# zjtggssg/ST-GCN-AltFormer

Measured on AMD Instinct MI355X. Metric: clips/sec ST-GCN forward, higher is better.
Workload: dtype bf16x3 (fp32 operands split hi+lo bf16, 3 MFMAs, fp32 accumulate); 1 GPU; SHREC-graph stem forward: V=22, T=180, 256 clips/GPU (BASELINE configs[1] batch at 1 GPU; weak-scaled); clips_per_gpu=256, global_clips=256, T=180, V=22, workload_key=256x180x22 bf16x3 fused nctv, csrc_digest=4cb53548ea740e3b, math=bf16x3, fused=True, layout=nctv, parallelism=dp1, parity=1e-4 rel fp32 vs CPU oracle (tests/test_gpu_parity.py)

## Files before the change

### st-gcn-altformer_amd/csrc/kf6.h

```cpp
#pragma once

#include <type_traits>

#include "bf16_common.h"

namespace stgcn {

namespace {

using namespace bf16k;

constexpr int NP6 = 256;
constexpr int NT6 = 256;
constexpr int KT6 = 9;
constexpr int FRAG6 = 1024;
constexpr int PAIR6 = 16 * FRAG6;
constexpr int RING6 = 3 * PAIR6;
constexpr int EPI6 = 4096;

using f32x4 = __attribute__((ext_vector_type(4))) float;
typedef __attribute__((address_space(3))) void *lptr6_t;

__device__ __forceinline__ void dma16v6(const void *g, unsigned lds_addr) {
    const unsigned lds = __builtin_amdgcn_readfirstlane(lds_addr);
    asm volatile("s_mov_b32 m0, %1\n\ts_nop 0\n\tglobal_load_lds_dwordx4 %0, off" : : "v"(g), "s"(lds) : "memory", "m0");
}
template <int N>
__device__ __forceinline__ void vm_wait_keep() { asm volatile("s_waitcnt vmcnt(%0)" ::"n"(N) : "memory"); }

struct FragB6 { uint4 hi[4], lo[4]; };

template <int I, int N, class F>
__device__ __forceinline__ void static_for(F &&f) {
    if constexpr (I < N) {
        f(std::integral_constant<int, I>{});
        static_for<I + 1, N>(f);
    }
}

struct TileInfo6 {
    int n, Vh, j0, half;
    TileGeomB g;
};

__device__ __forceinline__ float relu1(float x) {
    float r;
    asm("v_max_f32_e32 %0, 0, %1" : "=v"(r) : "v"(x));
    return r;
}

#ifdef STGCN_ABLATION
#define V6_STAMP(var) unsigned long long var = 0; if (dbg) { asm volatile("s_memtime %0\n\ts_waitcnt lgkmcnt(0)" : "=s"(var) :: "memory"); }
#define V6_ACC(slot, a, b) if (dbg) { tsum[slot] += (b) - (a); }
#else
#define V6_STAMP(var)
#define V6_ACC(slot, a, b)
#endif


template <bool NT>
__device__ __forceinline__ void st_out4(float *p, const float4 &v) {
#ifndef V6_PLAIN_STORES
    if constexpr (NT) {
        using f32x4v = __attribute__((ext_vector_type(4))) float;
        __builtin_nontemporal_store(f32x4v{v.x, v.y, v.z, v.w}, reinterpret_cast<f32x4v *>(p));
        return;
    }
#endif
    *reinterpret_cast<float4 *>(p) = v;
}

template <int TERMS, bool BF16OUT, bool WIDE>
__global__ __launch_bounds__(NT6) void stem_bf16_v6_kernel(
    const uint4 *__restrict__ pfrag, const float *__restrict__ x, int xsc, int xsp, const float *__restrict__ W12,
    const uint4 *__restrict__ Wp, const float *__restrict__ shift, void *y, int C, int T, int V, int ROWS,
    int tiles_per_clip, int ntiles, int abl, unsigned long long *dbg, int V0, int tpc1) {
#ifdef STGCN_ABLATION
    unsigned long long tsum[8] = {0, 0, 0, 0, 0, 0, 0, 0};
#endif
    extern __shared__ __attribute__((aligned(16))) char smem6[];
    const int tid = threadIdx.x;
    const int lane = tid & 63;
    const int wave = __builtin_amdgcn_readfirstlane(tid >> 6);
    const int TV = T * V;
    const int nch = C / CCB;
    const int npairs = nch * KT6 / 2;
    const int img_bytes = ROWS * PXB;
    const int buf_bytes = img_bytes * (TERMS == 3 ? 2 : 1);
    uint4 *W12q = reinterpret_cast<uint4 *>(smem6);
    char *ring = smem6 + C * W12P * 4;
    char *buf0 = ring + RING6;
    char *buf1 = buf0 + buf_bytes;
    uint4 *Fs = reinterpret_cast<uint4 *>(buf0 + max(2 * buf_bytes, 4 * EPI6));
    const uint4 *Pf = (WIDE && TERMS == 3) ? reinterpret_cast<const uint4 *>(buf1) : Fs + 4 * ROWS;
    const unsigned lds0 = (unsigned)(size_t)(lptr6_t)smem6;
    const unsigned ring_lds = lds0 + (unsigned)(ring - smem6);
    const unsigned pf_lds = lds0 + (unsigned)(reinterpret_cast<const char *>(Pf) - smem6);

    const int cg = blockIdx.y;
    const uint4 *wsrc = Wp + ((size_t)(cg * 8 + 2 * wave) * npairs * 2) * 64 + lane;
    auto dma_frag = [&](int qsrc, int slot, int d) {
        const int bw = d >> 1, img = d & 1;
        dma16v6(wsrc + ((size_t)(bw * npairs + qsrc) * 2 + img) * 64, ring_lds + slot * PAIR6 + ((2 * wave + bw) * 2 + img) * FRAG6);
    };
    auto tile_info = [&](int tile) {
        TileInfo6 ti;
        ti.n = tile / tiles_per_clip;
        const int r = tile - ti.n * tiles_per_clip;
        int idx;
        if (r < 2 * tpc1) { ti.half = r & 1; idx = r >> 1; }
        else { ti.half = 0; idx = r - tpc1; }
        ti.Vh = ti.half ? V - V0 : V0;
        ti.j0 = ti.half ? V0 : 0;
        ti.g = tile_geom_b(idx, ti.Vh, KT6, 1, T, NP6);
        return ti;
    };
    auto dma_pfrag = [&](int tile) {
        if constexpr (WIDE) {
            const TileInfo6 ti = tile_info(tile);
            const uint4 *src = pfrag + ((size_t)ti.n * 48 + ti.half * 24) * 64 + lane;
#pragma unroll
            for (int i = 0; i < 6; ++i) dma16v6(src + (wave + 4 * i) * 64, pf_lds + (wave + 4 * i) * FRAG6);
        } else {
            const int n = tile / tiles_per_clip;
            const uint4 *src = pfrag + (size_t)n * 12 * 64 + lane;
#pragma unroll
            for (int i = 0; i < 3; ++i) dma16v6(src + (wave + 4 * i) * 64, pf_lds + (wave + 4 * i) * FRAG6);
        }
    };

    struct XRegs { float xa[WIDE ? 16 : 8]; float xp[3]; };
    auto load_x = [&](XRegs &xr, int tile, int u) {
        int ln = tid & 63;
        asm volatile("" : "+v"(ln));
        const int mb = u >> 1, hh = u & 1;
        TileInfo6 ti;
        if constexpr (WIDE) ti = tile_info(tile);
        else {
            ti.n = tile / tiles_per_clip;
            ti.g = tile_geom_b(tile - ti.n * tiles_per_clip, V, KT6, 1, T, NP6);
        }
        const int n = ti.n;
        const TileGeomB g = ti.g;
        const __amdgpu_buffer_rsrc_t rs = __builtin_amdgcn_make_buffer_rsrc(
            const_cast<float *>(x + (size_t)n * 3 * TV), 0, (unsigned)(3 * TV * 4), 0x00020000);
        const int tf = g.t_first - (KT6 - 1) / 2 + 4 * mb;
        if constexpr (WIDE) {
            const int k = ln & 3, t = tf + ((ln & 15) >> 2), v0 = 8 * (ln >> 4);
            const bool okr = (k < 3) & (t >= 0) & (t < T);
            unsigned base = (unsigned)((k * xsc + (t * V + v0) * xsp) * 4);
            asm volatile("" : "+v"(base));
#pragma unroll
            for (int j = 0; j < 16; ++j) {
                const int dv = (j & 7) + 32 * (j >> 3);
                const unsigned off = (okr & (v0 + dv < V)) ? base + (unsigned)(dv * xsp * 4) : 0x7ffffff0u;
                xr.xa[j] = __builtin_bit_cast(float, __builtin_amdgcn_raw_buffer_load_b32(rs, off, 0, 0));
            }
            const int t2 = tf + (ln >> 4), w = 16 * hh + (ln & 15);
            const bool ok = (t2 >= 0) & (t2 < T) & (w < ti.Vh);
            unsigned base2 = (unsigned)(((t2 * V + ti.j0 + w) * xsp) * 4);
            asm volatile("" : "+v"(base2));
#pragma unroll
            for (int k2 = 0; k2 < 3; ++k2) {
                const unsigned off = ok ? base2 + (unsigned)(k2 * xsc * 4) : 0x7ffffff0u;
                xr.xp[k2] = __builtin_bit_cast(float, __builtin_amdgcn_raw_buffer_load_b32(rs, off, 0, 0));
            }
        } else {
            {
                const int k = ln & 3, t = tf + ((ln & 15) >> 2), v0 = 8 * (ln >> 4);
                const bool okr = k < 3 && t >= 0 && t < T;
#pragma unroll
                for (int j = 0; j < 8; ++j) {
                    const unsigned off = (okr && v0 + j < V) ? (unsigned)((k * xsc + (t * V + v0 + j) * xsp) * 4) : 0x7ffffff0u;
                    xr.xa[j] = __builtin_bit_cast(float, __builtin_amdgcn_raw_buffer_load_b32(rs, off, 0, 0));
                }
            }
            {
// ... 57 lines not shown
        const bool valid = p < g.span && gi >= 0 && gi < T * Vh;
        const float one = valid ? 1.f : 0.f;
        const float fa[8] = {d[0][0] * one, d[0][1] * one, d[0][2] * one, d[1][0] * one,
                             d[1][1] * one, d[1][2] * one, d[2][0] * one, d[2][1] * one};
        const float fb[8] = {d[2][2] * one, xr.xp[0] * one, xr.xp[1] * one, xr.xp[2] * one, one, 0.f, 0.f, 0.f};
        uint4 ha, la, hb, lb;
        split8(fa, ha, la);
        split8(fb, hb, lb);
        if (w < Vh && p < ROWS) {
            Fs[p] = ha;
            Fs[(size_t)ROWS + p] = hb;
            Fs[(size_t)2 * ROWS + p] = la;
            Fs[(size_t)3 * ROWS + p] = lb;
        }
    };
    auto feature_phase = [&](int tile, const XRegs &x0, const XRegs &x1, const XRegs &x2) {
        TileInfo6 ti;
        if constexpr (WIDE) ti = tile_info(tile);
        else {
            ti.n = tile / tiles_per_clip;
            ti.Vh = V;
            ti.j0 = ti.half = 0;
            ti.g = tile_geom_b(tile - ti.n * tiles_per_clip, V, KT6, 1, T, NP6);
        }
        const TileGeomB &g = ti.g;
        const int need = min(ROWS, ((g.span + 15) >> 4) << 4);
        const int nun = (((need + ti.Vh - 1) / ti.Vh + 3) >> 2) * 2;
        const bool two = ti.Vh > 16;
        for (int u = wave; u < nun; u += 4) {
            if (!two && (u & 1)) continue;
            if (u == wave) feature_unit(ti, u, x0);
            else if (u == wave + 4) feature_unit(ti, u, x1);
            else if (u == wave + 8) feature_unit(ti, u, x2);
            else {
                XRegs xr;
                load_x(xr, tile, u);
                feature_unit(ti, u, xr);
            }
        }
    };

    const int pl = lane & 15, pg = lane >> 4;
    struct Prod { uint4 wh, wl, fb; f32x4 d; int p; };
    auto prod_load = [&](Prod &pr, int ch, int bi) {
        pr.p = bi * 16 + pl;
        pr.wh = W12q[(size_t)(pg & 1) * C + ch * CCB + pl];
        pr.wl = W12q[(size_t)(2 + (pg & 1)) * C + ch * CCB + pl];
        pr.fb = Fs[(size_t)pg * ROWS + pr.p];
    };
    auto prod_mfma = [&](Prod &pr) {
        const bf16x8 f = __builtin_bit_cast(bf16x8, pr.fb);
        pr.d = f32x4{0.f, 0.f, 0.f, 0.f};
        pr.d = __builtin_amdgcn_mfma_f32_16x16x32_bf16(__builtin_bit_cast(bf16x8, pr.wh), f, pr.d, 0, 0, 0);
        pr.d = __builtin_amdgcn_mfma_f32_16x16x32_bf16(__builtin_bit_cast(bf16x8, pr.wl), f, pr.d, 0, 0, 0);
    };
    auto prod_mfma_slots = [&](Prod &pr) {
        using u32x4 = __attribute__((ext_vector_type(4))) unsigned;
        const u32x4 wh = __builtin_bit_cast(u32x4, pr.wh), wl = __builtin_bit_cast(u32x4, pr.wl), fb = __builtin_bit_cast(u32x4, pr.fb);
        asm volatile("v_mfma_f32_16x16x32_bf16 %0, %1, %2, 0" : "=&v"(pr.d) : "v"(wh), "v"(fb));
        asm volatile("v_mfma_f32_16x16x32_bf16 %0, %1, %2, %0" : "+v"(pr.d) : "v"(wl), "v"(fb));
    };
    auto prod_finish = [&](char *buf, const Prod &pr) {
        const float v0 = relu1(pr.d[0]), v1 = relu1(pr.d[1]), v2 = relu1(pr.d[2]), v3 = relu1(pr.d[3]);
        const unsigned h0 = pack_bf16x2(v0, v1), h1 = pack_bf16x2(v2, v3);
        const int off = lds_off(pr.p, pg >> 1) + (pg & 1) * 8;
        *reinterpret_cast<uint2 *>(buf + off) = make_uint2(h0, h1);
        if constexpr (TERMS == 3) {
            const unsigned l0 = pack_bf16x2(v0 - bf16_lo_to_f32(h0), v1 - bf16_hi_to_f32(h0));
            const unsigned l1 = pack_bf16x2(v2 - bf16_lo_to_f32(h1), v3 - bf16_hi_to_f32(h1));
            *reinterpret_cast<uint2 *>(buf + img_bytes + off) = make_uint2(l0, l1);
        }
    };

    for (int e = tid; e < C * 2; e += NT6) {
        const int c = e >> 1, kh = e & 1;
        float w8[8];
#pragma unroll
        for (int i = 0; i < 8; ++i) w8[i] = W12[c * W12P + kh * 8 + i];
        uint4 hi, lo;
        split8(w8, hi, lo);
        W12q[(size_t)kh * C + c] = hi;
        W12q[(size_t)(2 + kh) * C + c] = lo;
    }
    int tile = blockIdx.x;
    {
        XRegs x0 = {}, x1 = {}, x2 = {};
        if (tile < ntiles) {
            dma_pfrag(tile);
            load_x(x0, tile, wave);
            load_x(x1, tile, wave + 4);
            load_x(x2, tile, wave + 8);
        }
#pragma unroll
        for (int d = 0; d < 4; ++d) { dma_frag(0, 0, d); dma_frag(1, 1, d); }
        vm_wait_keep<0>();
        __syncthreads();
        if (tile < ntiles) feature_phase(tile, x0, x1, x2);
        __syncthreads();
    }

    int slot0 = 0, slot2 = 2, q2 = 2 % npairs;
    const int sel = lane >> 5, chh = (lane >> 4) & 1;
    for (; tile < ntiles; tile += gridDim.x) {
        TileInfo6 ti;
        if constexpr (WIDE) ti = tile_info(tile);
        else {
            ti.n = tile / tiles_per_clip;
            ti.Vh = V;
            ti.j0 = ti.half = 0;
            ti.g = tile_geom_b(tile - ti.n * tiles_per_clip, V, KT6, 1, T, NP6);
        }
        const int n = ti.n;
        const TileGeomB g = ti.g;
        const int Vh = ti.Vh;
        const int nblk = (g.span + 15) >> 4;
        const int next_tile = tile + gridDim.x;

        V6_STAMP(t_0)
        for (int b = wave; b < nblk; b += 4) {
            Prod pr;
            prod_load(pr, 0, b);
            prod_mfma(pr);
            prod_finish(buf0, pr);
        }
        unsigned boff[KT6];
        {
            const int q = g.q0 + wave * 64 + (lane & 15);
            const int prow = q - g.t_first * Vh;
#pragma unroll
            for (int tap = 0; tap < KT6; ++tap) boff[tap] = (unsigned)lds_off(prow + tap * Vh, chh);
        }
        f32x4 acc[8][4];
#pragma unroll
        for (int mb = 0; mb < 8; ++mb)
#pragma unroll
            for (int nb = 0; nb < 4; ++nb) acc[mb][nb] = f32x4{0.f, 0.f, 0.f, 0.f};
        __syncthreads();
        V6_STAMP(t_1)
        V6_ACC(0, t_0, t_1)

        auto rd = [&](const char *p) { return *reinterpret_cast<const uint4 *>(p); };
        auto load_b = [&](FragB6 &b, auto l0_c, auto nb_c, auto lo_c) {
            constexpr int l0 = decltype(l0_c)::value, l1 = l0 + 1, nb = decltype(nb_c)::value;
            constexpr bool lo_img = decltype(lo_c)::value;
            const char *b0 = (l0 >= KT6 ? buf1 : buf0), *b1 = (l1 >= KT6 ? buf1 : buf0);
            const unsigned o0 = boff[l0 % KT6], o1 = boff[l1 % KT6];
            const char *p = (sel ? b1 : b0) + (sel ? o1 : o0) + (nb * 16 * PXB) + (lo_img ? img_bytes : 0);
            if constexpr (lo_img) b.lo[nb] = rd(p); else b.hi[nb] = rd(p);
        };
        using IC0 = std::integral_constant<int, 0>;
        FragB6 b_cur = {}, b_nxt = {};
        uint4 ah0n = rd(ring + slot0 * PAIR6 + lane * 16), al0n = rd(ring + slot0 * PAIR6 + lane * 16 + FRAG6);
        static_for<0, 4>([&](auto nb_c) {
            load_b(b_cur, IC0{}, nb_c, std::false_type{});
            if constexpr (TERMS == 3) load_b(b_cur, IC0{}, nb_c, std::true_type{});
        });
        const int nper = nch / 2;
        for (int per = 0; per < nper; ++per) {
            if constexpr (!WIDE)
                if (per + 1 == nper && next_tile < ntiles) dma_pfrag(next_tile);
            static_for<0, 9>([&](auto pi_c) {
                constexpr int pi = decltype(pi_c)::value;
                constexpr int l0 = 2 * pi;
                constexpr int win = pi <= 2 ? 0 : (pi >= 5 && pi <= 7 ? 1 : -1);
                constexpr int wpi = win == 0 ? pi : pi - 5;
                constexpr int npb = win < 0 ? 0 : (wpi < 2 ? 3 : 2);
// ... 12 lines not shown
                int poff = 0;
                constexpr int NM = 32 * TERMS;
                auto filler = [&](auto v_c) {
                    constexpr int v = decltype(v_c)::value;
                    if constexpr (v % 12 == 2 && v / 12 < 7) ah[(v / 12 + 1) & 1] = rd(aslot + ((v / 12 + 1) * 2) * FRAG6);
                    if constexpr (TERMS == 3 && v % 12 == 3 && v / 12 < 7) al[(v / 12 + 1) & 1] = rd(aslot + ((v / 12 + 1) * 2 + 1) * FRAG6);
                    if constexpr (v >= 40 && v < 48) {
                        constexpr int nb = (v - 40) / 2;
                        constexpr int ln = (l0 + 2) % 18;
                        using LN = std::integral_constant<int, ln>;
                        using NB = std::integral_constant<int, nb>;
                        if constexpr (v % 2 == 0) load_b(b_nxt, LN{}, NB{}, std::false_type{});
                        else if constexpr (TERMS == 3) load_b(b_nxt, LN{}, NB{}, std::true_type{});
                    }
                    if constexpr (npb > 0 && v >= 8 && (v - 8) / 28 < npb) {
                        constexpr int b = (v - 8) / 28, w = (v - 8) % 28;
                        auto piece = [&]() {
                            if constexpr (w == 0) {
                                pr.p = min(wave + 4 * (3 * wpi + b), nblk - 1) * 16 + pl;
                                pr.wh = W12q[(size_t)(pg & 1) * C + pch * CCB + pl];
                            }
                            if constexpr (w == 1) pr.wl = W12q[(size_t)(2 + (pg & 1)) * C + pch * CCB + pl];
                            if constexpr (w == 2) pr.fb = Fs[(size_t)pg * ROWS + pr.p];
                            if constexpr (w == 10) { if constexpr (TERMS == 3) prod_mfma_slots(pr); else prod_mfma(pr); }
                            if constexpr (w == 14) {
                                pv0 = relu1(pr.d[0]); pv1 = relu1(pr.d[1]); pv2 = relu1(pr.d[2]); pv3 = relu1(pr.d[3]);
                            }
                            if constexpr (w == 15) { ph0 = pack_bf16x2(pv0, pv1); ph1 = pack_bf16x2(pv2, pv3); }
                            if constexpr (w == 16) poff = lds_off(pr.p, pg >> 1) + (pg & 1) * 8;
                            if constexpr (w == 17) *reinterpret_cast<uint2 *>(pbuf + poff) = make_uint2(ph0, ph1);
                            if constexpr (TERMS == 3 && w == 18) { pv0 -= bf16_lo_to_f32(ph0); pv1 -= bf16_hi_to_f32(ph0); }
                            if constexpr (TERMS == 3 && w == 19) { pv2 -= bf16_lo_to_f32(ph1); pv3 -= bf16_hi_to_f32(ph1); }
                            if constexpr (TERMS == 3 && w == 20) { ph0 = pack_bf16x2(pv0, pv1); ph1 = pack_bf16x2(pv2, pv3); }
                            if constexpr (TERMS == 3 && w == 21) *reinterpret_cast<uint2 *>(pbuf + img_bytes + poff) = make_uint2(ph0, ph1);
                        };
                        constexpr bool has_work = w <= 2 || w == 10 || (w >= 14 && w <= 17) || (TERMS == 3 && w >= 18 && w <= 21);
                        if constexpr (has_work) piece();
                    }
                    if constexpr (v >= 4 && v < 8) dma_frag(q2, slot2, v - 4);
                    if constexpr (v == 88) ah0n = rd(anext);
                    if constexpr (TERMS == 3 && v == 89) al0n = rd(anext + FRAG6);
                };
                static_for<0, NM>([&](auto i_c) {
                    constexpr int i = decltype(i_c)::value;
                    constexpr int mb = i / (4 * TERMS), nb = (i / TERMS) % 4, term = i % TERMS;
                    const bf16x8 a_h = __builtin_bit_cast(bf16x8, ah[mb & 1]), b_h = __builtin_bit_cast(bf16x8, b_cur.hi[nb]);
                    if constexpr (TERMS == 3) {
                        const bf16x8 a_l = __builtin_bit_cast(bf16x8, al[mb & 1]), b_l = __builtin_bit_cast(bf16x8, b_cur.lo[nb]);
                        if constexpr (term == 0) acc[mb][nb] = __builtin_amdgcn_mfma_f32_16x16x32_bf16(a_h, b_l, acc[mb][nb], 0, 0, 0);
                        else if constexpr (term == 1) acc[mb][nb] = __builtin_amdgcn_mfma_f32_16x16x32_bf16(a_l, b_h, acc[mb][nb], 0, 0, 0);
                        else acc[mb][nb] = __builtin_amdgcn_mfma_f32_16x16x32_bf16(a_h, b_h, acc[mb][nb], 0, 0, 0);
                    } else {
                        acc[mb][nb] = __builtin_amdgcn_mfma_f32_16x16x32_bf16(a_h, b_h, acc[mb][nb], 0, 0, 0);
                    }
                    if constexpr (term == TERMS - 1) asm volatile("" : "+a"(acc[mb][nb]));
#ifndef V6_NOFILL
                    static_for<i * (96 / NM), (i + 1) * (96 / NM)>(filler);
#endif
                    __builtin_amdgcn_sched_barrier(0);
                });
                b_cur = b_nxt;
                V6_STAMP(t_s1)
                V6_ACC((pi == 4 ? 6 : (pi == 0 ? 7 : (pi == 3 ? 5 : 4))), t_p0, t_s1)
                vm_wait_keep<0>();
                __syncthreads();
                V6_STAMP(t_s2)
                V6_ACC(2, t_s1, t_s2)
                slot0 = slot1;
                slot2 = slot2 == 2 ? 0 : slot2 + 1;
                q2 = q2 + 1 == npairs ? 0 : q2 + 1;
            });
        }
        vm_wait_keep<0>();
        V6_STAMP(t_2)
        V6_ACC(1, t_1, t_2)

        if constexpr (WIDE)
            if (next_tile < ntiles) dma_pfrag(next_tile);
        XRegs xn0, xn1, xn2;
        load_x(xn0, min(next_tile, ntiles - 1), wave);
        load_x(xn1, min(next_tile, ntiles - 1), wave + 4);
        load_x(xn2, min(next_tile, ntiles - 1), wave + 8);
        __builtin_amdgcn_sched_barrier(0);
        float *stg = reinterpret_cast<float *>(buf0 + wave * EPI6);
        const int qw = g.q0 + wave * 64;
        const bool full = g.q0 + NP6 - 1 <= g.q_last;
        if constexpr (WIDE) {
            auto clip_pixel = [&](int q) { const int t = q / Vh; return t * V + ti.j0 + (q - t * Vh); };
            if (abl & OPT_OUT_NTVC) {
                unsigned pt[4];
                bool pok[4];
#pragma unroll
                for (int it = 0; it < 4; ++it) {
                    const int q = qw + it * 16 + (lane >> 2);
                    pok[it] = q <= g.q_last;
                    pt[it] = (unsigned)(clip_pixel(min(q, g.q_last)) * C + 4 * (lane & 3));
                }
#pragma unroll
                for (int mb = 0; mb < 8; ++mb) {
                    const int ob = cg * 128 + mb * 16;
                    const float4 sh4 = *reinterpret_cast<const float4 *>(shift + ob + 4 * (lane >> 4));
#pragma unroll
                    for (int nb = 0; nb < 4; ++nb) {
                        const int px = nb * 16 + (lane & 15);
                        const float4 v = make_float4(fmaxf(acc[mb][nb][0] + sh4.x, 0.f), fmaxf(acc[mb][nb][1] + sh4.y, 0.f),
                                                     fmaxf(acc[mb][nb][2] + sh4.z, 0.f), fmaxf(acc[mb][nb][3] + sh4.w, 0.f));
                        *reinterpret_cast<float4 *>(stg + px * 16 + (((lane >> 4) ^ (px & 3)) << 2)) = v;
                    }
                    const size_t tbase = (size_t)n * TV * C + ob;
#pragma unroll
                    for (int it = 0; it < 4; ++it) {
                        const int idx = it * 64 + lane, px = idx >> 2, sl = idx & 3;
                        const float4 v = *reinterpret_cast<const float4 *>(stg + px * 16 + ((sl ^ (px & 3)) << 2));
                        if (pok[it]) {
                            if constexpr (BF16OUT)
                                *reinterpret_cast<uint2 *>(reinterpret_cast<unsigned short *>(y) + tbase + pt[it]) =
                                    make_uint2(pack_bf16x2(v.x, v.y), pack_bf16x2(v.z, v.w));
                            else
                                st_out4<false>(reinterpret_cast<float *>(y) + tbase + pt[it], v);
                        }
                    }
                }
            } else {
                const int qp = qw + 2 * (lane & 31);
                const bool pok = qp <= g.q_last;
                const unsigned lterm = (unsigned)((lane >> 5) * TV + clip_pixel(min(qp, g.q_last)));
#pragma unroll
                for (int mb = 0; mb < 8; ++mb) {
                    const int ob = cg * 128 + mb * 16;
                    const float4 sh4 = *reinterpret_cast<const float4 *>(shift + ob + 4 * (lane >> 4));
                    const float shv[4] = {sh4.x, sh4.y, sh4.z, sh4.w};
#pragma unroll
                    for (int nb = 0; nb < 4; ++nb)
#pragma unroll
                        for (int r = 0; r < 4; ++r)
                            stg[(4 * (lane >> 4) + r) * 64 + nb * 16 + (lane & 15)] = fmaxf(acc[mb][nb][r] + shv[r], 0.f);
                    const size_t tbase = ((size_t)n * C + ob) * TV;
#pragma unroll
                    for (int it = 0; it < 8; ++it) {
                        const float2 v = *reinterpret_cast<const float2 *>(stg + (it * 2 + (lane >> 5)) * 64 + 2 * (lane & 31));
                        const size_t sbase = tbase + (size_t)(it * 2) * TV;
                        if (pok) {
                            if constexpr (BF16OUT)
                                *reinterpret_cast<unsigned *>(reinterpret_cast<unsigned short *>(y) + sbase + lterm) = pack_bf16x2(v.x, v.y);
                            else
                                *reinterpret_cast<float2 *>(reinterpret_cast<float *>(y) + sbase + lterm) = v;
                        }
                    }
                }
            }
        } else if (abl & OPT_OUT_NTVC) {
            const unsigned lterm = (unsigned)((lane >> 2) * C + 4 * (lane & 3));
#pragma unroll
            for (int mb = 0; mb < 8; ++mb) {
                const int ob = cg * 128 + mb * 16;
                const float4 sh4 = *reinterpret_cast<const float4 *>(shift + ob + 4 * (lane >> 4));
#pragma unroll
                for (int nb = 0; nb < 4; ++nb) {
                    const int px = nb * 16 + (lane & 15);
                    const float4 v = make_float4(fmaxf(acc[mb][nb][0] + sh4.x, 0.f), fmaxf(acc[mb][nb][1] + sh4.y, 0.f),
                                                 fmaxf(acc[mb][nb][2] + sh4.z, 0.f), fmaxf(acc[mb][nb][3] + sh4.w, 0.f));
                    *reinterpret_cast<float4 *>(stg + px * 16 + (((lane >> 4) ^ (px & 3)) << 2)) = v;
                }
                const size_t tbase = ((size_t)n * TV + qw) * C + ob;
#pragma unroll
                for (int it = 0; it < 4; ++it) {
                    const int idx = it * 64 + lane, px = idx >> 2, sl = idx & 3;
                    const float4 v = *reinterpret_cast<const float4 *>(stg + px * 16 + ((sl ^ (px & 3)) << 2));
                    if (full || qw + px <= g.q_last) {
                        if constexpr (BF16OUT) {
                            unsigned short *yb = reinterpret_cast<unsigned short *>(y) + tbase + (size_t)(it * 16) * C;
                            *reinterpret_cast<uint2 *>(yb + lterm) = make_uint2(pack_bf16x2(v.x, v.y), pack_bf16x2(v.z, v.w));
                        } else {
                            float *yb = reinterpret_cast<float *>(y) + tbase + (size_t)(it * 16) * C;
                            st_out4<true>(yb + lterm, v);
                        }
                    }
                }
            }
        } else {
            const unsigned lterm = (unsigned)((lane >> 4) * TV + 4 * (lane & 15));
            const int c4l = 4 * (lane & 15);
#pragma unroll
            for (int mb = 0; mb < 8; ++mb) {
                const int ob = cg * 128 + mb * 16;
                const float4 sh4 = *reinterpret_cast<const float4 *>(shift + ob + 4 * (lane >> 4));
                const float shv[4] = {sh4.x, sh4.y, sh4.z, sh4.w};
#pragma unroll
                for (int nb = 0; nb < 4; ++nb)
#pragma unroll
                    for (int r = 0; r < 4; ++r)
                        stg[(4 * (lane >> 4) + r) * 64 + nb * 16 + (lane & 15)] = fmaxf(acc[mb][nb][r] + shv[r], 0.f);
                const size_t tbase = ((size_t)n * C + ob) * TV + qw;
                const bool al16 = ((tbase & 3) == 0) && (TV % 4 == 0);
#pragma unroll
                for (int it = 0; it < 4; ++it) {
                    const float4 v = *reinterpret_cast<const float4 *>(stg + (it * 4 + (lane >> 4)) * 64 + c4l);
                    const size_t sbase = tbase + (size_t)(it * 4) * TV;
                    if (full && al16) {
                        if constexpr (BF16OUT)
                            *reinterpret_cast<uint2 *>(reinterpret_cast<unsigned short *>(y) + sbase + lterm) =
                                make_uint2(pack_bf16x2(v.x, v.y), pack_bf16x2(v.z, v.w));
                        else
                            st_out4<true>(reinterpret_cast<float *>(y) + sbase + lterm, v);
                    } else {
                        const float e4[4] = {v.x, v.y, v.z, v.w};
#pragma unroll
                        for (int e = 0; e < 4; ++e)
                            if (qw + c4l + e <= g.q_last) store_out<BF16OUT>(y, sbase + lterm + e, e4[e]);
                    }
                }
            }
        }
        V6_STAMP(t_3)
        V6_ACC(3, t_2, t_3)
        if (next_tile < ntiles) {
            if constexpr (WIDE) {
                vm_wait_keep<0>();
                __syncthreads();
            }
            feature_phase(next_tile, xn0, xn1, xn2);
            V6_STAMP(t_4)
            __syncthreads();
        }
        V6_STAMP(t_5)
    }
#ifdef STGCN_ABLATION
    if (dbg && lane == 0 && blockIdx.x < 8 && blockIdx.y == 0)
        for (int i = 0; i < 8; ++i) dbg[(blockIdx.x * 8 + wave) * 8 + i] = tsum[i];
#endif
}

struct V6Plan {
    int rows = 0, tiles_per_clip = 0;
    size_t lds = 0;
    int v0 = 0, tpc1 = 0;
};

inline int v6_rows(int T, int Vh, int K) {
    int dt = ceil_div(NP6 - 1, Vh);
    if (dt > T - 1) dt = T - 1;
    const int span = (dt + K) * Vh;
    if (ceil_div(ceil_div(span, 16), 4) > 8) return 0;
    return (span + 15) / 16 * 16;
}

inline bool plan_v6_narrow(int C, int T, int V, int K, int terms, V6Plan &pl) {
    if (K != KT6 || C % 128 != 0 || V > 32) return false;
    const int rows = v6_rows(T, V, K);
    if (rows == 0) return false;
    const size_t buf = (size_t)rows * PXB * (terms == 3 ? 2 : 1);
    const size_t img = 2 * buf > (size_t)4 * EPI6 ? 2 * buf : (size_t)4 * EPI6;
    pl.lds = (size_t)C * W12P * 4 + RING6 + img + (size_t)rows * 64 + 12 * FRAG6;
    if (pl.lds > (size_t)kLdsBytes) return false;
    pl.rows = rows;
    pl.tiles_per_clip = ceil_div(T * V, NP6);
    return true;
}

inline bool plan_v6_wide(int C, int T, int V, int K, int terms, V6Plan &pl) {
    const int v0 = stem_wide_split(V);
    if (K != KT6 || C % 128 != 0 || v0 == 0) return false;
    const int r0 = v6_rows(T, v0, K), r1 = v6_rows(T, V - v0, K);
    if (r0 == 0 || r1 == 0) return false;
    const int rows = r0 > r1 ? r0 : r1;
    const size_t buf = (size_t)rows * PXB * (terms == 3 ? 2 : 1);
    const size_t img = 2 * buf > (size_t)4 * EPI6 ? 2 * buf : (size_t)4 * EPI6;
    if (terms == 3 && buf < (size_t)24 * FRAG6) return false;
    pl.lds = (size_t)C * W12P * 4 + RING6 + img + (size_t)rows * 64 + (terms == 3 ? 0 : 24 * FRAG6);
    if (pl.lds > (size_t)kLdsBytes) return false;
    pl.rows = rows;
    pl.v0 = v0;
    pl.tpc1 = ceil_div(T * (V - v0), NP6);
    pl.tiles_per_clip = ceil_div(T * v0, NP6) + pl.tpc1;
    return pl.tiles_per_clip - pl.tpc1 >= pl.tpc1;
}

template <bool WIDE>
bool stem_v6_form_supported(int C, int T, int V, int K, unsigned flags) {
    const unsigned math = flags & STGCN_MATH_MASK;
    if (math != STGCN_MATH_BF16X3 && math != STGCN_MATH_BF16) return false;
    const int terms = math == STGCN_MATH_BF16X3 ? 3 : 1;
    V6Plan pl;
    return T >= 1 && (WIDE ? plan_v6_wide(C, T, V, K, terms, pl) : plan_v6_narrow(C, T, V, K, terms, pl));
}

template <int TERMS, bool WIDE>
int launch_v6(const uint4 *pf, const float *x, int xsc, int xsp, const float *W12, const uint4 *Wq, const float *shift, void *y,
              int N, int C, int T, int V, const V6Plan &pl, bool bf16out, int opt, int num_cu, hipStream_t st) {
    const int ntiles = N * pl.tiles_per_clip;
    const dim3 grid(ntiles < num_cu ? ntiles : num_cu, C / 128, 1);
    auto kern = bf16out ? stem_bf16_v6_kernel<TERMS, true, WIDE> : stem_bf16_v6_kernel<TERMS, false, WIDE>;
    STGCN_HIP_CHECK(allow_lds(kern, pl.lds));
    hipLaunchKernelGGL(kern, grid, dim3(NT6), pl.lds, st, pf, x, xsc, xsp, W12, Wq, shift, y, C, T, V, pl.rows,
                       pl.tiles_per_clip, ntiles, opt, debug_buffer(), pl.v0, pl.tpc1);
    STGCN_LAUNCH_CHECK("stem_bf16_v6_kernel");
    return STGCN_OK;
}

template <bool WIDE>
int launch_stem_v6_form(const float *x, bool x_ntvc, const void *pfrag, const void *prep_w12, const void *Wq, const float *shift,
                        void *out, int N, int C, int T, int V, int K, unsigned flags, hipStream_t st) {
    const unsigned math = flags & STGCN_MATH_MASK;
    const int terms = math == STGCN_MATH_BF16X3 ? 3 : 1;
    const bool bf16out = (flags & STGCN_OUT_BF16) != 0;
    const int opt = (flags & STGCN_OUT_NTVC) ? OPT_OUT_NTVC : 0;
    V6Plan pl;
    if (!(WIDE ? plan_v6_wide(C, T, V, K, terms, pl) : plan_v6_narrow(C, T, V, K, terms, pl)))
        return fail(STGCN_ERR_UNSUPPORTED, "stem v6 kernel does not cover C=%d T=%d V=%d K=%d", C, T, V, K);
    if ((size_t)3 * T * V * 4 >= ((size_t)1 << 31) || (size_t)T * V * C >= ((size_t)1 << 31))
        return fail(STGCN_ERR_UNSUPPORTED, "stem v6: clip of T=%d V=%d exceeds a buffer resource", T, V);
    int dev = 0, num_cu = 256;
    STGCN_HIP_CHECK(hipGetDevice(&dev));
    STGCN_HIP_CHECK(hipDeviceGetAttribute(&num_cu, hipDeviceAttributeMultiprocessorCount, dev));
    const int xsc = x_ntvc ? 1 : T * V, xsp = x_ntvc ? 3 : 1;
    const uint4 *pf = (const uint4 *)pfrag;
    const float *W12 = (const float *)prep_w12;
    const uint4 *wq = (const uint4 *)Wq;
    return terms == 3 ? launch_v6<3, WIDE>(pf, x, xsc, xsp, W12, wq, shift, out, N, C, T, V, pl, bf16out, opt, num_cu, st)
                      : launch_v6<1, WIDE>(pf, x, xsc, xsp, W12, wq, shift, out, N, C, T, V, pl, bf16out, opt, num_cu, st);
}

}
}
```

### st-gcn-altformer_amd/csrc/stem_f16mx.hip

```cpp
#include "kf6.h"

namespace stgcn {

namespace {

using f16x8 = __attribute__((ext_vector_type(8))) _Float16;
using i32x8 = __attribute__((ext_vector_type(8))) int;

constexpr bool mx_slot_reg(int s) { return s >= 4 && (s >= 46 || (s - 4) % 3 == 0); }
constexpr int mx_index_reg(int s) { return s >= 46 ? 14 + (s - 46) : (s - 4) / 3; }
constexpr int hi_index_reg(int s) { return s < 4 ? s : 4 + 2 * ((s - 4) / 3) + ((s - 4) % 3 - 1); }
constexpr bool mx_slot_t8(int s) { return s >= 4 && (s >= 88 || (s - 4) % 3 != 2); }
constexpr int mx_index_t8(int s) { return s >= 88 ? 56 + (s - 88) : 2 * ((s - 4) / 3) + (s - 4) % 3; }
constexpr int hi_index_t8(int s) { return s < 4 ? s : 4 + (s - 4) / 3; }
template <bool BF16OUT>
__global__ __launch_bounds__(NT6) void stem_f16mx_kernel(
    const uint4 *__restrict__ pfrag, const float *__restrict__ x, int xsc, int xsp, const float *__restrict__ W12,
    const uint4 *__restrict__ Wp, const float *__restrict__ shift, void *y, int C, int T, int V, int ROWS,
    int tiles_per_clip, int ntiles, int abl, unsigned long long *dbg, const float *__restrict__ meta,
    const float *__restrict__ bounds) {
    constexpr int TERMS = 3;
#ifdef STGCN_ABLATION
    unsigned long long tsum[8] = {0, 0, 0, 0, 0, 0, 0, 0};
#endif
// ... 512 lines not shown
        if ((threadIdx.x & 63) == 0) red[i][threadIdx.x >> 6] = m[i];
    }
    __syncthreads();
    if (threadIdx.x == 0) {
        float r[6];
        for (int i = 0; i < 6; ++i) r[i] = fmaxf(fmaxf(red[i][0], red[i][1]), fmaxf(red[i][2], red[i][3]));
        for (int i = 0; i < 5; ++i) meta[i] = r[i];
        int e = (int)((__float_as_uint(r[5]) >> 23) & 0xffu) - 126;
        e = max(-90, min(90, e));
        e = max(-60, min(60, e));
        meta[5] = (float)(14 - e);
        meta[6] = meta[7] = 0.f;
    }
}

__device__ __forceinline__ unsigned e4m3_of(float v) { return (unsigned)__builtin_amdgcn_cvt_pk_fp8_f32(v, 0.f, 0, false) & 0xffu; }

__global__ void f16mx_pack_kernel(const float *__restrict__ W, const float *__restrict__ scale, const float *__restrict__ meta,
                                  uint4 *__restrict__ Wq, int Cin, int Cout) {
    const size_t e = (size_t)blockIdx.x * 256 + threadIdx.x;
    const int npairs = Cin / CCB * KT6 / 2;
    if (e >= (size_t)(Cout / 16) * npairs * 2 * 64) return;
    const int l = (int)(e & 63), img = (int)((e >> 6) & 1);
    const int q = (int)((e >> 7) % npairs), obg = (int)((e >> 7) / npairs);
    const int ob = obg & 7, cg = obg >> 3;
    const float sW = exp2f(meta[5]);
    constexpr float sWH = 0.015625f, sWL = 32.f;
    auto wv = [&](int o, int c, int tap) { return scale[o] * W[((size_t)o * Cin + c) * KT6 + tap] * sW; };
    unsigned out[4] = {0, 0, 0, 0};
    if (img == 0) {
        const int o = obg * 16 + (l & 15), f = 2 * q + (l >> 5);
        const int c0 = (f / KT6) * CCB + 8 * ((l >> 4) & 1), tap = f % KT6;
#pragma unroll
        for (int j = 0; j < 4; ++j) {
            const _Float16 a = (_Float16)wv(o, c0 + 2 * j, tap), b = (_Float16)wv(o, c0 + 2 * j + 1, tap);
            out[j] = (unsigned)__builtin_bit_cast(unsigned short, a) | ((unsigned)__builtin_bit_cast(unsigned short, b) << 16);
        }
    } else {
        const int pi = q % 9, per = q / 9;
        int o, chunk, tap, term;
        if (pi != 4) {
            const int ci = pi < 4 ? pi : pi - 5;
            term = ci >> 1;
            const int mb = 4 * (ci & 1) + (ob >> 1), half = ob & 1;
            chunk = 2 * per + (pi > 4 ? 1 : 0);
            o = cg * 128 + mb * 16 + (l & 15);
            tap = 2 * (l >> 4) + half;
        } else {
            const int op = 2 * ob + (l >> 5), u16 = l & 31;
            term = op >> 3;
            o = cg * 128 + (op & 7) * 16 + (u16 >> 1);
            chunk = 2 * per + (u16 & 1);
            tap = 8;
        }
#pragma unroll
        for (int k = 0; k < 16; ++k) {
            const float w = wv(o, chunk * CCB + k, tap);
            const float wh = (float)(_Float16)w;
            const unsigned b = term == 0 ? e4m3_of((w - wh) * sWL) : e4m3_of(wh * sWH);
            out[k >> 2] |= b << (8 * (k & 3));
        }
    }
    Wq[e] = make_uint4(out[0], out[1], out[2], out[3]);
}

int launch_v7(const uint4 *pf, const float *x, int xsc, int xsp, const float *W12, const uint4 *Wq, const float *shift, void *y,
              int N, int C, int T, int V, const V6Plan &pl, bool bf16out, int opt, int num_cu, const float *meta,
              const float *bounds, hipStream_t st) {
    const int ntiles = N * pl.tiles_per_clip;
    const dim3 grid(ntiles < num_cu ? ntiles : num_cu, C / 128, 1);
    auto kern = bf16out ? stem_f16mx_kernel<true> : stem_f16mx_kernel<false>;
    STGCN_HIP_CHECK(allow_lds(kern, pl.lds));
    hipLaunchKernelGGL(kern, grid, dim3(NT6), pl.lds, st, pf, x, xsc, xsp, W12, Wq, shift, y, C, T, V, pl.rows,
                       pl.tiles_per_clip, ntiles, opt, debug_buffer(), meta, bounds);
    STGCN_LAUNCH_CHECK("stem_f16mx_kernel");
    return STGCN_OK;
}

}

bool stem_f16mx_supported(int C, int T, int V, int K, unsigned flags) {
    if ((flags & STGCN_MATH_MASK) != STGCN_MATH_BF16X3 || !(flags & STGCN_STEM_F16MX)) return false;
    V6Plan pl;
    return T >= 1 && plan_v6_narrow(C, T, V, K, 3, pl);
}

size_t stem_f16mx_prep_bytes(int C, int K) { return 256 + (size_t)C * C * K * 4; }

int launch_stem_f16mx_prepare(const float *W12, const float *Wt, const float *t_scale, void *dst, int C, hipStream_t st) {
    float *meta = (float *)dst;
    hipLaunchKernelGGL(f16mx_meta_kernel, dim3(1), dim3(256), 0, st, W12, Wt, t_scale, meta, C, C);
    STGCN_LAUNCH_CHECK("f16mx_meta_kernel");
    const size_t units = (size_t)(C / 16) * (C / CCB * KT6 / 2) * 2 * 64;
    hipLaunchKernelGGL(f16mx_pack_kernel, dim3((unsigned)((units + 255) / 256)), dim3(256), 0, st, Wt, t_scale, meta,
                       (uint4 *)((char *)dst + 256), C, C);
    STGCN_LAUNCH_CHECK("f16mx_pack_kernel");
    return STGCN_OK;
}

int launch_stem_f16mx(const float *x, bool x_ntvc, const void *pfrag, const void *bounds, const void *prep_w12, const void *mx_blob,
                      const float *shift, void *out, int N, int C, int T, int V, int K, unsigned flags, hipStream_t st) {
    const bool bf16out = (flags & STGCN_OUT_BF16) != 0;
    const int opt = (flags & STGCN_OUT_NTVC) ? OPT_OUT_NTVC : 0;
    V6Plan pl;
    if (!plan_v6_narrow(C, T, V, K, 3, pl))
        return fail(STGCN_ERR_UNSUPPORTED, "stem f16mx kernel does not cover C=%d T=%d V=%d K=%d", C, T, V, K);
    if ((size_t)3 * T * V * 4 >= ((size_t)1 << 31))
        return fail(STGCN_ERR_UNSUPPORTED, "stem f16mx: clip of T=%d V=%d exceeds a buffer resource", T, V);
    int dev = 0, num_cu = 256;
    STGCN_HIP_CHECK(hipGetDevice(&dev));
    STGCN_HIP_CHECK(hipDeviceGetAttribute(&num_cu, hipDeviceAttributeMultiprocessorCount, dev));
    const int xsc = x_ntvc ? 1 : T * V, xsp = x_ntvc ? 3 : 1;
    return launch_v7((const uint4 *)pfrag, x, xsc, xsp, (const float *)prep_w12, (const uint4 *)((const char *)mx_blob + 256), shift,
                     out, N, C, T, V, pl, bf16out, opt, num_cu, (const float *)mx_blob, (const float *)bounds, st);
}

}
```

Before: 375,000 clips/s.

## Software-pipeline stem epilogue with LDS shift cache and double-buffered staging

The epilogue now caches the per-block shift vector in LDS once per block rather than reading it from global memory for every output block. It stages the next channel block into LDS while the current one is being stored, using two staging slices per wave in the narrow path. It also splits each store loop into compile-time fast (full tile) and slow (bounds-checked) variants, and XOR-swizzles the row staging to cut bank conflicts. The price is extra LDS (a larger staging area plus a shift buffer), which could cut occupancy or make plan_v6 reject some shapes, and the code gets more complex.

```diff
diff --git a/st-gcn-altformer_amd/csrc/kf6.h b/st-gcn-altformer_amd/csrc/kf6.h
--- a/st-gcn-altformer_amd/csrc/kf6.h
+++ b/st-gcn-altformer_amd/csrc/kf6.h
@@ -17,6 +17,7 @@
 constexpr int PAIR6 = 16 * FRAG6;
 constexpr int RING6 = 3 * PAIR6;
 constexpr int EPI6 = 4096;
+constexpr int SHB6 = 512;
 
 using f32x4 = __attribute__((ext_vector_type(4))) float;
 typedef __attribute__((address_space(3))) void *lptr6_t;
@@ -37,6 +38,36 @@
         static_for<I + 1, N>(f);
     }
 }
+
+template <class AccRow>
+__device__ __forceinline__ void stage_rows6(float *stg, const AccRow &a, const float4 &sh4, float lo, int lane) {
+    const int g = lane >> 4, s = (g & 1) * 16;
+    float *we = stg + g * 256 + (lane & 15) + s, *wo = stg + g * 256 + (lane & 15) - s;
+    const float shv[4] = {sh4.x, sh4.y, sh4.z, sh4.w};
+#pragma unroll
+    for (int nb = 0; nb < 4; ++nb)
+#pragma unroll
+        for (int r = 0; r < 4; ++r) ((nb & 1) ? wo : we)[r * 64 + nb * 16] = fmaxf(a[nb][r] + shv[r], lo);
+}
+__device__ __forceinline__ float4 staged_row4(const float *stg, int it, int lane) {
+    return *reinterpret_cast<const float4 *>(stg + (it * 4 + (lane >> 4)) * 64 + ((4 * (lane & 15)) ^ ((it & 1) << 4)));
+}
+__device__ __forceinline__ void fill_shift6(float *shs, const float *__restrict__ shift, int n, int tid) {
+    if (tid < 128) shs[tid] = tid < n ? shift[tid] : 0.f;
+}
+
+struct V6Carve { int buf0, fs, pf, sh, total; };
+__host__ __device__ inline V6Carve v6_carve(int C, int rows, int terms, bool wide, int stg) {
+    const int buf = rows * PXB * (terms == 3 ? 2 : 1);
+    V6Carve c;
+    c.buf0 = C * W12P * 4 + RING6;
+    c.fs = c.buf0 + (2 * buf > stg ? 2 * buf : stg);
+    c.pf = (wide && terms == 3) ? c.buf0 + buf : c.fs + rows * 64;
+    c.sh = c.fs + rows * 64 + (wide ? (terms == 3 ? 0 : 24 * FRAG6) : 12 * FRAG6);
+    c.total = c.sh + SHB6;
+    return c;
+}
+constexpr int stg_bytes6(bool wide) { return (wide ? 4 : 8) * EPI6; }
 
 struct TileInfo6 {
     int n, Vh, j0, half;
@@ -87,12 +118,14 @@
     const int npairs = nch * KT6 / 2;
     const int img_bytes = ROWS * PXB;
     const int buf_bytes = img_bytes * (TERMS == 3 ? 2 : 1);
+    const V6Carve cv = v6_carve(C, ROWS, TERMS, WIDE, stg_bytes6(WIDE));
     uint4 *W12q = reinterpret_cast<uint4 *>(smem6);
     char *ring = smem6 + C * W12P * 4;
-    char *buf0 = ring + RING6;
+    char *buf0 = smem6 + cv.buf0;
     char *buf1 = buf0 + buf_bytes;
-    uint4 *Fs = reinterpret_cast<uint4 *>(buf0 + max(2 * buf_bytes, 4 * EPI6));
-    const uint4 *Pf = (WIDE && TERMS == 3) ? reinterpret_cast<const uint4 *>(buf1) : Fs + 4 * ROWS;
+    uint4 *Fs = reinterpret_cast<uint4 *>(smem6 + cv.fs);
+    const uint4 *Pf = reinterpret_cast<const uint4 *>(smem6 + cv.pf);
+    float *shs = reinterpret_cast<float *>(smem6 + cv.sh);
     const unsigned lds0 = (unsigned)(size_t)(lptr6_t)smem6;
     const unsigned ring_lds = lds0 + (unsigned)(ring - smem6);
     const unsigned pf_lds = lds0 + (unsigned)(reinterpret_cast<const char *>(Pf) - smem6);
@@ -316,6 +349,7 @@
         W12q[(size_t)kh * C + c] = hi;
         W12q[(size_t)(2 + kh) * C + c] = lo;
     }
+    fill_shift6(shs, shift + blockIdx.y * 128, 128, tid);
     int tile = blockIdx.x;
     {
         XRegs x0 = {}, x1 = {}, x2 = {};
@@ -494,9 +528,30 @@
         load_x(xn1, min(next_tile, ntiles - 1), wave + 4);
         load_x(xn2, min(next_tile, ntiles - 1), wave + 8);
         __builtin_amdgcn_sched_barrier(0);
-        float *stg = reinterpret_cast<float *>(buf0 + wave * EPI6);
+        constexpr int NSL = stg_bytes6(WIDE) / (4 * EPI6);
+        float *stg = reinterpret_cast<float *>(buf0 + wave * (NSL * EPI6));
+        const float4 *shs4 = reinterpret_cast<const float4 *>(shs) + (lane >> 4);
         const int qw = g.q0 + wave * 64;
         const bool full = g.q0 + NP6 - 1 <= g.q_last;
+        using FastT = std::true_type;
+        using SlowT = std::false_type;
+        auto stage_px = [&](float *sl, int mb, const float4 &sh4) {
+#pragma unroll
+            for (int nb = 0; nb < 4; ++nb) {
+                const int px = nb * 16 + (lane & 15);
+                const float4 v = make_float4(fmaxf(acc[mb][nb][0] + sh4.x, 0.f), fmaxf(acc[mb][nb][1] + sh4.y, 0.f),
+                                             fmaxf(acc[mb][nb][2] + sh4.z, 0.f), fmaxf(acc[mb][nb][3] + sh4.w, 0.f));
+                *reinterpret_cast<float4 *>(sl + px * 16 + (((lane >> 4) ^ (px & 3)) << 2)) = v;
+            }
+        };
+        auto staged_px4 = [&](const float *sl, int it) {
+            const int idx = it * 64 + lane, px = idx >> 2, slot = idx & 3;
+            return *reinterpret_cast<const float4 *>(sl + px * 16 + ((slot ^ (px & 3)) << 2));
+        };
+        if (abl & OPT_OUT_NTVC) stage_px(stg, 0, shs4[0]);
+        else stage_rows6(stg, acc[0], shs4[0], 0.f, lane);
+        float4 sh = shs4[4];
+        asm volatile("" : : "v"(xn2.xp[2]));
         if constexpr (WIDE) {
             auto clip_pixel = [&](int q) { const int t = q / Vh; return t * V + ti.j0 + (q - t * Vh); };
             if (abl & OPT_OUT_NTVC) {
@@ -508,121 +563,132 @@
                     pok[it] = q <= g.q_last;
                     pt[it] = (unsigned)(clip_pixel(min(q, g.q_last)) * C + 4 * (lane & 3));
                 }
-#pragma unroll
-                for (int mb = 0; mb < 8; ++mb) {
-                    const int ob = cg * 128 + mb * 16;
-                    const float4 sh4 = *reinterpret_cast<const float4 *>(shift + ob + 4 * (lane >> 4));
-#pragma unroll
-                    for (int nb = 0; nb < 4; ++nb) {
-                        const int px = nb * 16 + (lane & 15);
-                        const float4 v = make_float4(fmaxf(acc[mb][nb][0] + sh4.x, 0.f), fmaxf(acc[mb][nb][1] + sh4.y, 0.f),
-                                                     fmaxf(acc[mb][nb][2] + sh4.z, 0.f), fmaxf(acc[mb][nb][3] + sh4.w, 0.f));
-                        *reinterpret_cast<float4 *>(stg + px * 16 + (((lane >> 4) ^ (px & 3)) << 2)) = v;
-                    }
-                    const size_t tbase = (size_t)n * TV * C + ob;
-#pragma unroll
-                    for (int it = 0; it < 4; ++it) {
-                        const int idx = it * 64 + lane, px = idx >> 2, sl = idx & 3;
-                        const float4 v = *reinterpret_cast<const float4 *>(stg + px * 16 + ((sl ^ (px & 3)) << 2));
-                        if (pok[it]) {
-                            if constexpr (BF16OUT)
-                                *reinterpret_cast<uint2 *>(reinterpret_cast<unsigned short *>(y) + tbase + pt[it]) =
-                                    make_uint2(pack_bf16x2(v.x, v.y), pack_bf16x2(v.z, v.w));
-                            else
-                                st_out4<false>(reinterpret_cast<float *>(y) + tbase + pt[it], v);
+                auto blocks = [&](auto fast_c) {
+                    constexpr bool FAST = decltype(fast_c)::value;
+#pragma unroll
+                    for (int mb = 0; mb < 8; ++mb) {
+                        const int ob = cg * 128 + mb * 16;
+                        if (mb > 0) stage_px(stg, mb, sh);
+                        if (mb > 0 && mb < 7) sh = shs4[4 * (mb + 1)];
+                        const size_t tbase = (size_t)n * TV * C + ob;
+                        float4 v[4];
+#pragma unroll
+                        for (int it = 0; it < 4; ++it) v[it] = staged_px4(stg, it);
+#pragma unroll
+                        for (int it = 0; it < 4; ++it) {
+                            if (FAST || pok[it]) {
+                                if constexpr (BF16OUT)
+                                    *reinterpret_cast<uint2 *>(reinterpret_cast<unsigned short *>(y) + tbase + pt[it]) =
+                                        make_uint2(pack_bf16x2(v[it].x, v[it].y), pack_bf16x2(v[it].z, v[it].w));
+                                else
+                                    st_out4<false>(reinterpret_cast<float *>(y) + tbase + pt[it], v[it]);
+                            }
                         }
                     }
-                }
+                };
+                if (full) blocks(FastT{}); else blocks(SlowT{});
             } else {
                 const int qp = qw + 2 * (lane & 31);
                 const bool pok = qp <= g.q_last;
                 const unsigned lterm = (unsigned)((lane >> 5) * TV + clip_pixel(min(qp, g.q_last)));
+                auto blocks = [&](auto fast_c) {
+                    constexpr bool FAST = decltype(fast_c)::value;
+#pragma unroll
+                    for (int mb = 0; mb < 8; ++mb) {
+                        const int ob = cg * 128 + mb * 16;
+                        if (mb > 0) stage_rows6(stg, acc[mb], sh, 0.f, lane);
+                        if (mb > 0 && mb < 7) sh = shs4[4 * (mb + 1)];
+                        const size_t tbase = ((size_t)n * C + ob) * TV;
+                        float2 v[8];
+#pragma unroll
+                        for (int it = 0; it < 8; ++it)
+                            v[it] = *reinterpret_cast<const float2 *>(stg + (it * 2 + (lane >> 5)) * 64 + ((2 * (lane & 31)) ^ ((it & 2) << 3)));
+#pragma unroll
+                        for (int it = 0; it < 8; ++it) {
+                            const size_t sbase = tbase + (size_t)(it * 2) * TV;
+                            if (FAST || pok) {
+                                if constexpr (BF16OUT)
+                                    *reinterpret_cast<unsigned *>(reinterpret_cast<unsigned short *>(y) + sbase + lterm) = pack_bf16x2(v[it].x, v[it].y);
+                                else
+                                    *reinterpret_cast<float2 *>(reinterpret_cast<float *>(y) + sbase + lterm) = v[it];
+                            }
+                        }
+                    }
+                };
+                if (full) blocks(FastT{}); else blocks(SlowT{});
+            }
+        } else if (abl & OPT_OUT_NTVC) {
+            const unsigned lterm = (unsigned)((lane >> 2) * C + 4 * (lane & 3));
+            auto blocks = [&](auto fast_c) {
+                constexpr bool FAST = decltype(fast_c)::value;
 #pragma unroll
                 for (int mb = 0; mb < 8; ++mb) {
                     const int ob = cg * 128 + mb * 16;
-                    const float4 sh4 = *reinterpret_cast<const float4 *>(shift + ob + 4 * (lane >> 4));
-                    const float shv[4] = {sh4.x, sh4.y, sh4.z, sh4.w};
-#pragma unroll
-                    for (int nb = 0; nb < 4; ++nb)
-#pragma unroll
-                        for (int r = 0; r < 4; ++r)
-                            stg[(4 * (lane >> 4) + r) * 64 + nb * 16 + (lane & 15)] = fmaxf(acc[mb][nb][r] + shv[r], 0.f);
-                    const size_t tbase = ((size_t)n * C + ob) * TV;
-#pragma unroll
-                    for (int it = 0; it < 8; ++it) {
-                        const float2 v = *reinterpret_cast<const float2 *>(stg + (it * 2 + (lane >> 5)) * 64 + 2 * (lane & 31));
-                        const size_t sbase = tbase + (size_t)(it * 2) * TV;
-                        if (pok) {
-                            if constexpr (BF16OUT)
-                                *reinterpret_cast<unsigned *>(reinterpret_cast<unsigned short *>(y) + sbase + lterm) = pack_bf16x2(v.x, v.y);
-                            else
-                                *reinterpret_cast<float2 *>(reinterpret_cast<float *>(y) + sbase + lterm) = v;
+                    float *sl = stg + (mb % NSL) * (EPI6 / 4);
+                    if (mb > 0) stage_px(sl, mb, sh);
+                    if (mb > 0 && mb < 7) sh = shs4[4 * (mb + 1)];
+                    const size_t tbase = ((size_t)n * TV + qw) * C + ob;
+                    float4 v[4];
+#pragma unroll
+                    for (int it = 0; it < 4; ++it) v[it] = staged_px4(sl, it);
+#pragma unroll
+                    for (int it = 0; it < 4; ++it) {
+                        const int px = (it * 64 + lane) >> 2;
+                        if (FAST || qw + px <= g.q_last) {
+                            if constexpr (BF16OUT) {
+                                unsigned short *yb = reinterpret_cast<unsigned short *>(y) + tbase + (size_t)(it * 16) * C;
+                                *reinterpret_cast<uint2 *>(yb + lterm) = make_uint2(pack_bf16x2(v[it].x, v[it].y), pack_bf16x2(v[it].z, v[it].w));
+                            } else {
+                                float *yb = reinterpret_cast<float *>(y) + tbase + (size_t)(it * 16) * C;
+                                st_out4<true>(yb + lterm, v[it]);
+                            }
                         }
                     }
                 }
-            }
-        } else if (abl & OPT_OUT_NTVC) {
-            const unsigned lterm = (unsigned)((lane >> 2) * C + 4 * (lane & 3));
-#pragma unroll
-            for (int mb = 0; mb < 8; ++mb) {
-                const int ob = cg * 128 + mb * 16;
-                const float4 sh4 = *reinterpret_cast<const float4 *>(shift + ob + 4 * (lane >> 4));
-#pragma unroll
-                for (int nb = 0; nb < 4; ++nb) {
-                    const int px = nb * 16 + (lane & 15);
-                    const float4 v = make_float4(fmaxf(acc[mb][nb][0] + sh4.x, 0.f), fmaxf(acc[mb][nb][1] + sh4.y, 0.f),
-                                                 fmaxf(acc[mb][nb][2] + sh4.z, 0.f), fmaxf(acc[mb][nb][3] + sh4.w, 0.f));
-                    *reinterpret_cast<float4 *>(stg + px * 16 + (((lane >> 4) ^ (px & 3)) << 2)) = v;
-                }
-                const size_t tbase = ((size_t)n * TV + qw) * C + ob;
-#pragma unroll
-                for (int it = 0; it < 4; ++it) {
-                    const int idx = it * 64 + lane, px = idx >> 2, sl = idx & 3;
-                    const float4 v = *reinterpret_cast<const float4 *>(stg + px * 16 + ((sl ^ (px & 3)) << 2));
-                    if (full || qw + px <= g.q_last) {
-                        if constexpr (BF16OUT) {
-                            unsigned short *yb = reinterpret_cast<unsigned short *>(y) + tbase + (size_t)(it * 16) * C;
-                            *reinterpret_cast<uint2 *>(yb + lterm) = make_uint2(pack_bf16x2(v.x, v.y), pack_bf16x2(v.z, v.w));
-                        } else {
-                            float *yb = reinterpret_cast<float *>(y) + tbase + (size_t)(it * 16) * C;
-                            st_out4<true>(yb + lterm, v);
-                        }
-                    }
-                }
-            }
+            };
+            if (full) blocks(FastT{}); else blocks(SlowT{});
         } else {
             const unsigned lterm = (unsigned)((lane >> 4) * TV + 4 * (lane & 15));
             const int c4l = 4 * (lane & 15);
-#pragma unroll
-            for (int mb = 0; mb < 8; ++mb) {
-                const int ob = cg * 128 + mb * 16;
-                const float4 sh4 = *reinterpret_cast<const float4 *>(shift + ob + 4 * (lane >> 4));
-                const float shv[4] = {sh4.x, sh4.y, sh4.z, sh4.w};
-#pragma unroll
-                for (int nb = 0; nb < 4; ++nb)
-#pragma unroll
-                    for (int r = 0; r < 4; ++r)
-                        stg[(4 * (lane >> 4) + r) * 64 + nb * 16 + (lane & 15)] = fmaxf(acc[mb][nb][r] + shv[r], 0.f);
-                const size_t tbase = ((size_t)n * C + ob) * TV + qw;
-                const bool al16 = ((tbase & 3) == 0) && (TV % 4 == 0);
-#pragma unroll
-                for (int it = 0; it < 4; ++it) {
-                    const float4 v = *reinterpret_cast<const float4 *>(stg + (it * 4 + (lane >> 4)) * 64 + c4l);
-                    const size_t sbase = tbase + (size_t)(it * 4) * TV;
-                    if (full && al16) {
-                        if constexpr (BF16OUT)
-                            *reinterpret_cast<uint2 *>(reinterpret_cast<unsigned short *>(y) + sbase + lterm) =
-                                make_uint2(pack_bf16x2(v.x, v.y), pack_bf16x2(v.z, v.w));
-                        else
-                            st_out4<true>(reinterpret_cast<float *>(y) + sbase + lterm, v);
+            const size_t tbase0 = ((size_t)n * C + cg * 128) * TV + qw;
+            const bool al16 = ((tbase0 & 3) == 0) && (TV % 4 == 0);
+            auto blocks = [&](auto fast_c) {
+                constexpr bool FAST = decltype(fast_c)::value;
+#pragma unroll
+                for (int mb = 0; mb < 8; ++mb) {
+                    float *sl = stg + (mb % NSL) * (EPI6 / 4);
+                    if (mb > 0) stage_rows6(sl, acc[mb], sh, 0.f, lane);
+                    if (mb > 0 && mb < 7) sh = shs4[4 * (mb + 1)];
+                    const size_t tbase = tbase0 + (size_t)(mb * 16) * TV;
+                    unsigned lt = lterm;
+                    int c4 = c4l;
+                    if constexpr (!FAST) asm volatile("" : "+v"(lt), "+v"(c4));
+                    auto row = [&](int it, const float4 &vv) {
+                        const size_t sbase = tbase + (size_t)(it * 4) * TV;
+                        if constexpr (FAST) {
+                            if constexpr (BF16OUT)
+                                *reinterpret_cast<uint2 *>(reinterpret_cast<unsigned short *>(y) + sbase + lt) =
+                                    make_uint2(pack_bf16x2(vv.x, vv.y), pack_bf16x2(vv.z, vv.w));
+                            else
+                                st_out4<true>(reinterpret_cast<float *>(y) + sbase + lt, vv);
+                        } else {
+                            const float e4[4] = {vv.x, vv.y, vv.z, vv.w};
+#pragma unroll
+                            for (int e = 0; e < 4; ++e)
+                                if (qw + c4 + e <= g.q_last) store_out<BF16OUT>(y, sbase + lt + e, e4[e]);
+                        }
+                    };
+                    if constexpr (FAST) {
+                        const float4 v0 = staged_row4(sl, 0, lane), v1 = staged_row4(sl, 1, lane), v2 = staged_row4(sl, 2, lane),
+                                     v3 = staged_row4(sl, 3, lane);
+                        row(0, v0); row(1, v1); row(2, v2); row(3, v3);
                     } else {
-                        const float e4[4] = {v.x, v.y, v.z, v.w};
-#pragma unroll
-                        for (int e = 0; e < 4; ++e)
-                            if (qw + c4l + e <= g.q_last) store_out<BF16OUT>(y, sbase + lterm + e, e4[e]);
+#pragma unroll
+                        for (int it = 0; it < 4; ++it) row(it, staged_row4(sl, it, lane));
                     }
                 }
-            }
+            };
+            if (full && al16) blocks(FastT{}); else blocks(SlowT{});
         }
         V6_STAMP(t_3)
         V6_ACC(3, t_2, t_3)
@@ -657,13 +723,11 @@
     return (span + 15) / 16 * 16;
 }
 
-inline bool plan_v6_narrow(int C, int T, int V, int K, int terms, V6Plan &pl) {
+inline bool plan_v6_narrow(int C, int T, int V, int K, int terms, V6Plan &pl, int stg = stg_bytes6(false)) {
     if (K != KT6 || C % 128 != 0 || V > 32) return false;
     const int rows = v6_rows(T, V, K);
     if (rows == 0) return false;
-    const size_t buf = (size_t)rows * PXB * (terms == 3 ? 2 : 1);
-    const size_t img = 2 * buf > (size_t)4 * EPI6 ? 2 * buf : (size_t)4 * EPI6;
-    pl.lds = (size_t)C * W12P * 4 + RING6 + img + (size_t)rows * 64 + 12 * FRAG6;
+    pl.lds = (size_t)v6_carve(C, rows, terms, false, stg).total;
     if (pl.lds > (size_t)kLdsBytes) return false;
     pl.rows = rows;
     pl.tiles_per_clip = ceil_div(T * V, NP6);
@@ -677,9 +741,8 @@
     if (r0 == 0 || r1 == 0) return false;
     const int rows = r0 > r1 ? r0 : r1;
     const size_t buf = (size_t)rows * PXB * (terms == 3 ? 2 : 1);
-    const size_t img = 2 * buf > (size_t)4 * EPI6 ? 2 * buf : (size_t)4 * EPI6;
-    if (terms == 3 && buf < (size_t)24 * FRAG6) return false;
-    pl.lds = (size_t)C * W12P * 4 + RING6 + img + (size_t)rows * 64 + (terms == 3 ? 0 : 24 * FRAG6);
+    if (terms == 3 && (buf < (size_t)24 * FRAG6 || buf < (size_t)stg_bytes6(true))) return false;
+    pl.lds = (size_t)v6_carve(C, rows, terms, true, stg_bytes6(true)).total;
     if (pl.lds > (size_t)kLdsBytes) return false;
     pl.rows = rows;
     pl.v0 = v0;
diff --git a/st-gcn-altformer_amd/csrc/stem_f16mx.hip b/st-gcn-altformer_amd/csrc/stem_f16mx.hip
--- a/st-gcn-altformer_amd/csrc/stem_f16mx.hip
+++ b/st-gcn-altformer_amd/csrc/stem_f16mx.hip
@@ -618,7 +618,7 @@
 bool stem_f16mx_supported(int C, int T, int V, int K, unsigned flags) {
     if ((flags & STGCN_MATH_MASK) != STGCN_MATH_BF16X3 || !(flags & STGCN_STEM_F16MX)) return false;
     V6Plan pl;
-    return T >= 1 && plan_v6_narrow(C, T, V, K, 3, pl);
+    return T >= 1 && plan_v6_narrow(C, T, V, K, 3, pl, 4 * EPI6);
 }
 
 size_t stem_f16mx_prep_bytes(int C, int K) { return 256 + (size_t)C * C * K * 4; }
@@ -639,7 +639,7 @@
     const bool bf16out = (flags & STGCN_OUT_BF16) != 0;
     const int opt = (flags & STGCN_OUT_NTVC) ? OPT_OUT_NTVC : 0;
     V6Plan pl;
-    if (!plan_v6_narrow(C, T, V, K, 3, pl))
+    if (!plan_v6_narrow(C, T, V, K, 3, pl, 4 * EPI6))
         return fail(STGCN_ERR_UNSUPPORTED, "stem f16mx kernel does not cover C=%d T=%d V=%d K=%d", C, T, V, K);
     if ((size_t)3 * T * V * 4 >= ((size_t)1 << 31))
         return fail(STGCN_ERR_UNSUPPORTED, "stem f16mx: clip of T=%d V=%d exceeds a buffer resource", T, V);
```

Result: no change. 377,200 clips/s, median of 6 (+0.6%).
